# miaoyin390/DNN-Compression-Tensor-ADMM

Measured on AMD Instinct MI355X. Metric: ADMM projection iters/sec (all layers) + per-layer SVD GFLOP/s, ResNet-50 TT ranks, higher is better.
Workload: dtype f32 (Gram, eigen-solve and its filter products accumulate in f64); 1 GPU; resnet50_tt: 34 layers, 20099072 weights, hp table tt_resnet50_hp.HyperParamsDictGeneralRatio3x; tables=1, parallelism=layer-shard x1 (latency-model partition, one scalar all-reduce per step)

## Files before the change

### dnn-compression-tensor-admm_amd/csrc/filter.hip

```cpp
#include "common.h"

namespace tadmm {

typedef double double2v_t __attribute__((ext_vector_type(2)));
constexpr int kMomParts = 64;

__device__ __forceinline__ double hash_unit(uint32_t a, uint32_t b) {
  uint64_t x = ((uint64_t)a << 32) ^ (uint64_t)b;
  x += 0x9E3779B97F4A7C15ull;
  x = (x ^ (x >> 30)) * 0xBF58476D1CE4E5B9ull;
  x = (x ^ (x >> 27)) * 0x94D049BB133111EBull;
  x ^= x >> 31;
  return (double)(int64_t)(x >> 11) * (1.0 / 4503599627370496.0) - 1.0;
}

__global__ __launch_bounds__(256) void filt_init_kernel(const FiltProb* __restrict__ probs,
                                                        const BlockRef* __restrict__ map, int test_zero_col) {
  const BlockRef br = map[blockIdx.x];
  const FiltProb p = probs[br.prob];
  if (br.local == 0 && threadIdx.x == 0) {
    FiltState* st = p.st;
    st->base = 0; st->res = 1; st->nsteps = 0; st->active = 1; st->alive = 1; st->bad = 0; st->stage = 0;
    st->products = 2;
    st->products_fast = 0; st->precise_stages = 0; st->logamp_precise = 0.0;
// ... 4 lines not shown
  const int64_t total = (int64_t)p.rp * p.ldy;
  const int64_t i0 = ((int64_t)br.local * 256 + threadIdx.x) * 4;
  double* Y = p.ring[0];
#pragma unroll
  for (int u = 0; u < 4; ++u) {
    const int64_t i = i0 + u;
    if (i < total) {
      const int col = (int)(i % p.ldy);
      Y[i] = (col < p.N && col != test_zero_col) ? hash_unit((uint32_t)br.prob * 2654435761u + 17u, (uint32_t)i) : 0.0;
    }
  }
}

__device__ __forceinline__ double acosh_pos(double x) { return log(x + sqrt(fmax(x * x - 1.0, 0.0))); }

__global__ __launch_bounds__(256) void filt_plan_kernel(const FiltProb* __restrict__ probs, FiltParams prm,
                                                        int last_stage, int stage_fast, int* __restrict__ verdict) {
  __shared__ double rho[256], sorted[256];
  const FiltProb p = probs[blockIdx.x];
  FiltState* st = p.st;
  const int tid = threadIdx.x;
  if (st->bad || !st->active) {
    __syncthreads();
    if (tid == 0) {
      st->nsteps = 0; st->res = st->base; st->active = 0;
      if (st->bad) { st->alive = 0; *p.skip_slot = 1; }
      verdict[1 + blockIdx.x] = 0;
    }
    return;
  }
  const int rp = p.rp;
  for (int j = tid; j < rp; j += 256) {
    double v = 0.0;
    for (int t = 0; t < p.rq_tiles; ++t) v += p.rqpart[(int64_t)t * rp + j];
    rho[j] = v;
  }
  __syncthreads();
  for (int j = tid; j < rp; j += 256) {
    const double v = rho[j];
    int rank = 0;
    for (int i = 0; i < rp; ++i) {
      const double w = rho[i];
      rank += (w > v) || (w == v && i < j);
    }
    sorted[rank] = v;
  }
  __syncthreads();
  if (tid == 0) {
    const double l1 = sorted[0], lr = sorted[p.r - 1], b = sorted[rp - 1];
    bool ok = isfinite(l1) && isfinite(b) && b > 0.0 && lr > b * (1.0 + 1e-9) && l1 >= lr;
    int m = 0;
    bool more = false;
    if (ok) {
      const double e = 0.5 * b, c = 0.5 * b;
      const double xr = (lr - c) / e, x1 = (l1 - c) / e;
      const double ar = acosh_pos(xr), a1 = acosh_pos(x1);
      double need = prm.log_target - st->logamp;
      if (st->products_fast > 0 || (stage_fast & 1)) need = fmax(need, prm.log_precise - st->logamp_precise);
      if (need > 0.0) {
        const double ln2 = 0.6931471805599453;
        const double cmax = st->stage == 0 ? fmin(prm.cond_max, prm.cond_first) : prm.cond_max;
        int mc = (int)floor(log(2.0 * cmax) / a1);
        mc = max(1, mc);
        int mn = (int)ceil((need + ln2) / ar);
        mn = max(1, mn);
        m = min(prm.max_degree, min(mc, mn));
        st->logamp += m * ar - ln2;
        st->coef1[0] = 1.0 / e; st->coef1[1] = -c / e;
        st->coefk[0] = 2.0 / e; st->coefk[1] = -2.0 * c / e; st->coefk[2] = -1.0;
        if (!(stage_fast & 1)) { st->precise_stages += 1; st->logamp_precise += m * ar - ln2; }
        double after = prm.log_target - st->logamp;
        if (st->products_fast > 0 || (stage_fast & 1)) after = fmax(after, prm.log_precise - st->logamp_precise);
        more = after > 0.0;
      }
      st->b = b; st->lr = lr; st->l1 = l1;
    } else {
      st->bad = 1; st->alive = 0; *p.skip_slot = 1;
    }
    st->nsteps = m;
    st->products += (m > 0) ? m : 1;
    if (stage_fast & 1) st->products_fast += (m > 0) ? m : 1;
    if ((stage_fast & 2) && st->stage == 0) st->products_fast += 1;
    int res = st->base + m;
    res -= (res >= 3) ? 3 : 0; res -= (res >= 3) ? 3 : 0; res -= (res >= 3) ? 3 : 0;
    st->res = res % 3;
    st->active = (m > 0 && more && !last_stage) ? 1 : 0;
    st->stage += 1;
    verdict[1 + blockIdx.x] = (m > 0 ? 1 : 0) | (st->active ? 2 : 0);
  }
}

__global__ void filt_flags_kernel(const FiltProb* __restrict__ probs, int nprob) {
  const int q = blockIdx.x * blockDim.x + threadIdx.x;
  if (q >= nprob) return;
  const FiltProb p = probs[q];
  if (p.st->bad) { p.st->alive = 0; *p.skip_slot = 1; }
}

__global__ __launch_bounds__(256) void filt_theta_kernel(const FiltProb* __restrict__ probs) {
  const FiltProb p = probs[blockIdx.x];
  if (p.st->bad) return;
  for (int c = threadIdx.x; c < p.r32; c += 256) {
    const double s = c < p.r ? p.sigma[c] : 0.0;
    p.theta[c] = s * s;
  }
}

__global__ __launch_bounds__(256) void filt_verdict_kernel(const FiltProb* __restrict__ probs, FiltParams prm,
                                                           int* __restrict__ verdict) {
  __shared__ double part[256];
  const FiltProb p = probs[blockIdx.x];
  FiltState* st = p.st;
  const int tid = threadIdx.x;
  if (st->bad) {
    if (tid == 0) { verdict[1 + blockIdx.x] = 0; *p.fb_skip = 0; }
    return;
  }
  const double th_next = p.lam[p.order[p.r]];
  double acc = 0.0;
  for (int c = tid; c < p.r; c += 256) {
    double rn = 0.0;
    for (int t = 0; t < p.v_tiles; ++t) rn += p.vpart[(int64_t)t * p.r32 + c];
    const double gap = p.theta[c] - th_next;
    acc += (gap > 0.0) ? rn / (gap * gap) : INFINITY;
  }
  part[tid] = acc;
  __syncthreads();
  for (int o = 128; o > 0; o >>= 1) {
    if (tid < o) part[tid] += part[tid + o];
    __syncthreads();
  }
  if (tid == 0) {
    const double crit = sqrt(part[0]);
    st->crit = crit;
    const double th_r = p.theta[p.r - 1];
    bool guard_ok = !(st->guard > th_r * (1.0 + 1e-9)) && st->guard == st->guard;
    if (st->mom_on) {
      double m[5] = {0.0, 0.0, 0.0, 0.0, 0.0};
      for (int w = 0; w < kMomParts; ++w)
        for (int q = 0; q < 5; ++q) m[q] += st->mom[w * 5 + q];
      const double trd = m[1] - m[4], d2 = m[0] - 2.0 * m[2] + m[3];
      const double bound = trd > 0.0 ? d2 / trd : 0.0;
      if (bound > th_r * (1.0 + 1e-6) || bound != bound) guard_ok = false;
      st->guard = fmax(st->guard, bound);
    }
    const bool ok = crit <= prm.sin_tol && guard_ok;
    if (!ok) { st->bad = 1; st->alive = 0; }
    *p.fb_skip = ok ? 1 : 0;
    verdict[1 + blockIdx.x] = ok ? 1 : 0;
  }
}

__global__ __launch_bounds__(256) void filt_moments_kernel(const FiltProb* __restrict__ probs) {
  __shared__ double red[5][4];
  const FiltProb p = probs[blockIdx.x];
  FiltState* st = p.st;
  if (st->bad) return;
  const int part = blockIdx.y, tid = threadIdx.x, lane = tid & 63, wave = tid >> 6;
  int tb = st->base + 1;
  tb -= tb >= 3 ? 3 : 0;
  auto sumsq = [&](const double* __restrict__ a, int64_t total) {
    const int64_t per = ((total / kMomParts + 511) / 512) * 512;
    const int64_t lo = (int64_t)part * per, hi = lo + per < total ? lo + per : total;
    double s0 = 0.0, s1 = 0.0, s2 = 0.0, s3 = 0.0;
    for (int64_t i = lo + 2 * tid; i < hi; i += 2048) {
      double2v_t v0 = {0, 0}, v1 = {0, 0}, v2 = {0, 0}, v3 = {0, 0};
      v0 = *reinterpret_cast<const double2v_t*>(a + i);
      if (i + 512 < hi) v1 = *reinterpret_cast<const double2v_t*>(a + i + 512);
      if (i + 1024 < hi) v2 = *reinterpret_cast<const double2v_t*>(a + i + 1024);
      if (i + 1536 < hi) v3 = *reinterpret_cast<const double2v_t*>(a + i + 1536);
      s0 += v0.x * v0.x + v0.y * v0.y; s1 += v1.x * v1.x + v1.y * v1.y;
      s2 += v2.x * v2.x + v2.y * v2.y; s3 += v3.x * v3.x + v3.y * v3.y;
    }
    return (s0 + s1) + (s2 + s3);
  };
  const double g2 = sumsq(p.G, (int64_t)p.Npad * p.ldg);
  const double t2 = sumsq(p.ring[tb], (int64_t)p.rp * p.ldy);
  const double h2 = sumsq(p.H, (int64_t)p.rp * p.ldh);
  double tg = 0.0, th = 0.0;
  if (part == 0) {
    for (int i = tid; i < p.N; i += 256) tg += p.G[(int64_t)i * p.ldg + i];
    for (int j = tid; j < p.rp; j += 256) th += p.H[(int64_t)j * p.ldh + j];
  }
  double v[5] = {g2, tg, t2, h2, th};
#pragma unroll
  for (int q = 0; q < 5; ++q) {
#pragma unroll
    for (int o = 32; o > 0; o >>= 1) v[q] += __shfl_xor(v[q], o, 64);
    if (lane == 0) red[q][wave] = v[q];
  }
  __syncthreads();
  if (tid < 5) st->mom[part * 5 + tid] = (red[tid][0] + red[tid][1]) + (red[tid][2] + red[tid][3]);
  if (part == 0 && tid == 0) st->mom_on = 1;
}

__global__ __launch_bounds__(1024) void filt_guard_kernel(const FiltProb* __restrict__ probs, int nsteps) {
  extern __shared__ __attribute__((aligned(16))) double gsm[];
  __shared__ double red[16];
  const FiltProb p = probs[blockIdx.x];
  FiltState* st = p.st;
  if (st->bad) return;
  const int N = p.N, Npad = p.Npad, rp = p.rp, ldy = p.ldy, ldg = p.ldg;
  const double* __restrict__ Q = p.ring[st->base];
  const double* __restrict__ G = p.G;
  double* z = gsm;
  double* w = z + Npad;
  double* c = w + Npad;
  double* pacc = c + rp;
  const int tid = threadIdx.x, lane = tid & 63, wave = tid >> 6;
  auto wave_sum = [&](double v) {
#pragma unroll
    for (int o = 32; o > 0; o >>= 1) v += __shfl_xor(v, o, 64);
    return v;
  };
  auto block_sum = [&](double v) {
    v = wave_sum(v);
    __syncthreads();
    if (lane == 0) red[wave] = v;
// ... 81 lines not shown
    project(w);
    double a = 0.0, b = 0.0;
    for (int i = tid; i < N; i += 1024) { a += z[i] * w[i]; b += w[i] * w[i]; }
    rho = fmax(rho, block_sum(a));
    const double n2 = block_sum(b);
    if (!(n2 > 0.0)) break;
    const double inv = 1.0 / sqrt(n2);
    for (int i = tid; i < N; i += 1024) z[i] = w[i] * inv;
    __syncthreads();
  }
  if (tid == 0) st->guard = rho;
}

__global__ __launch_bounds__(256) void filt_emit_kernel(const FiltProb* __restrict__ probs,
                                                        const BlockRef* __restrict__ map) {
  const BlockRef br = map[blockIdx.x];
  const FiltProb p = probs[br.prob];
  if (p.st->bad) return;
  const int lane = threadIdx.x & 63, wave = threadIdx.x >> 6;
  const int c = br.local * 4 + wave;
  if (c >= p.r) return;
  const double* row = p.UT + (int64_t)c * p.ldy;
  const int N = p.N;
  double best = -1.0; int besti = 0;
  double nrm = 0.0;
  for (int i = lane; i < N; i += 64) {
    const double v = row[i], a = fabs(v);
    nrm += v * v;
    if (a > best) { best = a; besti = i; }
  }
#pragma unroll
  for (int o = 32; o > 0; o >>= 1) {
    const double ob = __shfl_down(best, o, 64);
    const int oi = __shfl_down(besti, o, 64);
    nrm += __shfl_xor(nrm, o, 64);
    if (ob > best || (ob == best && oi < besti)) { best = ob; besti = oi; }
  }
  besti = __shfl(besti, 0, 64);
  const double sgn = (row[besti] < 0.0) ? -1.0 : 1.0;
  const double inv = nrm > 0.0 ? sgn / sqrt(nrm) : 0.0;
  const double sig = p.sigma[c];
  const double isig = sig > 0.0 ? 1.0 / sig : 0.0;
  const int R = p.ldo ? p.ldo : p.r;
  for (int i = lane; i < N; i += 64) {
    const double v = row[i] * inv;
    if (p.mode == 0) {
      p.out_a[(int64_t)i * R + c] = (float)v;
    } else if (p.mode == 1) {
      p.out_a[(int64_t)i * R + c] = (float)(v * isig);
      p.out_b[(int64_t)c * N + i] = (float)(v * sig);
    } else if (p.mode == 3) {
      p.out_a[(int64_t)i * R + c] = (float)(v * isig);
    }
  }
}

void launch_filt_init(const FiltProb* probs_dev, const BlockRef* map_dev, int nblocks, int nprob, hipStream_t s) {
  if (nblocks <= 0) return;
  int zero_col = -1;
  if (const char* e = getenv("TADMM_FILTER_TEST_ZERO_COL")) zero_col = atoi(e);
  hipLaunchKernelGGL(filt_init_kernel, dim3(nblocks), dim3(256), 0, s, probs_dev, map_dev, zero_col);
}
void launch_filt_moments(const FiltProb* probs_dev, int nprob, hipStream_t s) {
  if (nprob <= 0) return;
  hipLaunchKernelGGL(filt_moments_kernel, dim3(nprob, kMomParts), dim3(256), 0, s, probs_dev);
}
void launch_filt_guard(const FiltProb* probs_dev, int nprob, int npad_max, int rp_max, int steps, hipStream_t s) {
// ... 28 lines not shown
```

### dnn-compression-tensor-admm_amd/csrc/filter_host.h

```cpp
#pragma once
#include <memory>
#include "host.h"

namespace tadmm {

static inline int filter_block_size(int N, int r) {
  const char* e = getenv("TADMM_FILTER");
  if (e && !atoi(e)) return 0;
  int min_n = 192;
  if (const char* m = getenv("TADMM_FILTER_MINN")) min_n = atoi(m);
  if (N < min_n || r < 16) return 0;
  double over = 1.45;
  if (const char* o = getenv("TADMM_FILTER_OVERSAMPLE")) over = atof(o);
  int rp = (int)align_up((size_t)(over * r + 0.999), 32);
  double min_over = 1.15;
  if (const char* o = getenv("TADMM_FILTER_MIN_OVERSAMPLE")) min_over = atof(o);
  if (rp > 256) {
    rp = 256;
    if ((double)rp < min_over * r) return 0;
  }
  if (rp * 100 > 56 * N || rp <= r) return 0;
  return rp;
}

// ... 495 lines not shown
    if (fg.side->ok && hipEventRecord(fg.side->fork, s) == hipSuccess &&
        hipStreamWaitEvent(fg.side->st, fg.side->fork, 0) == hipSuccess) {
      launch_filt_guard(probs, fg.nf, fg.npad_max, fg.rp_max, filter_guard_steps(), fg.side->st);
      fg.guard_forked = hipEventRecord(fg.side->join, fg.side->st) == hipSuccess;
    }
  }
  gemm(fg.tfinal);
  gemm(fg.hform);
  if (filter_moments_on()) launch_filt_moments(probs, fg.nf, s);
  if (debug) fprintf(stderr, "[tadmm] filter: %d problems, %d stages of <= %d steps, product tiles %d x %d (%d blocks a launch)\n", fg.nf, stages,
                     fg.max_degree, fg.tile_m, filter_tile_n(), fg.p1.nblocks);
  return TADMM_OK;
}

static inline int filter_run_post(tadmm_handle h, FilterGroup& fg, char* ws, PollCtx& poll, hipStream_t s, bool debug,
                                  int* nbad, FilterTiming* tm = nullptr) {
  *nbad = 0;
  if (fg.nf == 0) return TADMM_OK;
  auto D = [&](size_t off) { return ws + off; };
  const FiltProb* probs = (const FiltProb*)D(fg.prob_off);
  const FiltParams prm = filter_params(fg);
  launch_filt_theta(probs, fg.nf, s);
  if (fg.guard_forked) HIP_OK(h, hipStreamWaitEvent(s, fg.side->join, 0));
  else launch_filt_guard(probs, fg.nf, fg.npad_max, fg.rp_max, filter_guard_steps(), s);
  launch_dgemm((const DgemmDesc*)D(fg.uform.desc_off), (const BlockRef*)D(fg.uform.map_off), fg.uform.nblocks, false, s);
  {
    const bool t = tm && tm->on;
    if (t) (void)hipEventRecord(tm->a, s);
    launch_dgemm_nt64((const DgemmDesc*)D(fg.verify.desc_off), (const BlockRef*)D(fg.verify.map_off), fg.verify.nblocks, s, filter_tile_n(), fg.tile_m);
    if (t) {
      float ms = 0.f;
// ... 4 lines not shown
    }
  }
  if (fg.ncomp > 0) {
    const CompDesc* cd = (const CompDesc*)D(fg.comp_off);
    launch_comp_form(cd, (const BlockRef*)D(fg.cform.map_off), fg.cform.nblocks, s);
    for (int pass = 0; pass < 2; ++pass) {
      launch_dgemm_nt64((const DgemmDesc*)D(fg.cgram.desc_off), (const BlockRef*)D(fg.cgram.map_off), fg.cgram.nblocks, s, filter_tile_n(), fg.tile_m);
      launch_chol_factor((const CholDesc*)D(fg.cchol_off), fg.ncomp, s);
      launch_chol_solve((const CholDesc*)D(fg.cchol_off), (const BlockRef*)D(fg.csolve_map_off), fg.csolve_blocks, s);
    }
  }
  launch_filt_verdict(probs, fg.nf, prm, poll.host, s);
  launch_filt_emit(probs, (const BlockRef*)D(fg.emit.map_off), fg.emit.nblocks, s);
  if (fg.ncomp > 0) launch_comp_emit((const CompDesc*)D(fg.comp_off), (const BlockRef*)D(fg.cemit.map_off), fg.cemit.nblocks, s);
  HIP_OK(h, hipEventRecord(poll.ev[0], s));
  HIP_OK(h, hipEventSynchronize(poll.ev[0]));
  int bad = 0;
  for (int q = 0; q < fg.nf; ++q) bad += poll.host[1 + q] ? 0 : 1;
  *nbad = bad;
  fg.last_bad = bad;
  if (tm && tm->on) {
    std::vector<FiltProb> hp(fg.nf);
    if (hipMemcpy(hp.data(), probs, hp.size() * sizeof(FiltProb), hipMemcpyDeviceToHost) == hipSuccess) {
      for (int q = 0; q < fg.nf; ++q) {
        FiltState st;
        if (hipMemcpy(&st, hp[q].st, sizeof st, hipMemcpyDeviceToHost) != hipSuccess) break;
        const double rp = hp[q].rp, np = hp[q].Npad, r32 = hp[q].r32;
        const double stages = st.stage;
        tm->fast_flops += 2.0 * rp * np * np * st.products_fast;
        tm->gemm_flops += 2.0 * rp * np * np * (st.products - st.products_fast)
// ... 22 lines not shown
```

### dnn-compression-tensor-admm_amd/csrc/gram.hip

```cpp
#include "common.h"
#include <type_traits>

namespace tadmm {

typedef double double4_t __attribute__((ext_vector_type(4)));

__device__ __forceinline__ double4_t mfma_f64(double a, double b, double4_t c) {
  return __builtin_amdgcn_mfma_f64_16x16x4f64(a, b, c, 0, 0, 0);
}

__device__ __forceinline__ void tile_pair(int tp, int nt, int& ti, int& tj) {
  int a = 0, rowlen = nt;
  while (tp >= rowlen) { tp -= rowlen; ++a; --rowlen; }
  ti = a; tj = a + tp;
}

__global__ __launch_bounds__(256) void gram_partial_kernel(const GramDesc* __restrict__ descs,
                                                           const BlockRef* __restrict__ map,
                                                           const int32_t* __restrict__ skip) {
  __shared__ double red[4][4][64 * 4];
  __shared__ double tile[32][33];
  const BlockRef br = map[blockIdx.x];
  if (skip && skip[br.prob]) return;
  const GramDesc d = descs[br.prob];
// ... 148 lines not shown
    G[(int64_t)(ti * 32 + rr) * gld + tj * 32 + cc] = tile[rr][cc];
    if (!diag) G[(int64_t)(tj * 32 + rr) * gld + ti * 32 + cc] = tile[cc][rr];
  }
  if (tj == d.nt - 1) {
    const int padw = d.ld - d.Npad;
    for (int e = threadIdx.x; e < 32 * padw; e += 256) {
      const int rr = e / padw, cc = e - rr * padw;
      G[(int64_t)(ti * 32 + rr) * gld + d.Npad + cc] = 0.0;
    }
  }
}

__global__ __launch_bounds__(256) void gram_reduce_kernel(const GramDesc* __restrict__ descs,
                                                          const BlockRef* __restrict__ map,
                                                          const int32_t* __restrict__ skip) {
  const BlockRef br = map[blockIdx.x];
  if (skip && skip[br.prob]) return;
  const GramDesc d = descs[br.prob];
  const int ntp = d.nt * (d.nt + 1) / 2;
  const int64_t total = (int64_t)d.Npad * d.ld;
  const int64_t base = (int64_t)br.local * 1024;
  for (int t = threadIdx.x; t < 1024; t += 256) {
    const int64_t idx = base + t;
    if (idx >= total) break;
    const int j = (int)(idx / d.ld), i = (int)(idx - (int64_t)j * d.ld);
    double v = 0.0;
    if (j < d.N && i < d.N) {
      int a = j >> 5, b = i >> 5, jr = j & 31, ir = i & 31;
      if (a > b) { int s = a; a = b; b = s; s = jr; jr = ir; ir = s; }
      if (a == b && jr > ir) { const int s = jr; jr = ir; ir = s; }
      const int tp = a * d.nt - (a * (a - 1)) / 2 + (b - a);
      const double* p = d.partial + (int64_t)tp * 1024 + jr * 32 + ir;
      const int64_t stride = (int64_t)ntp * 1024;
      int ks = 0;
      for (; ks + 8 <= d.ksplit; ks += 8) {
        double t[8];
#pragma unroll
        for (int u = 0; u < 8; ++u) t[u] = p[(ks + u) * stride];
        v += ((t[0] + t[1]) + (t[2] + t[3])) + ((t[4] + t[5]) + (t[6] + t[7]));
      }
      for (; ks < d.ksplit; ++ks) v += p[ks * stride];
    }
    d.G[idx] = v;
  }
}

void launch_gram_partial(const GramDesc* descs_dev, const BlockRef* map_dev, int nblocks, hipStream_t s,
                         const int32_t* skip) {
  if (nblocks <= 0) return;
  hipLaunchKernelGGL(gram_partial_kernel, dim3(nblocks), dim3(256), 0, s, descs_dev, map_dev, skip);
}

void launch_gram_reduce(const GramDesc* descs_dev, const BlockRef* map_dev, int nblocks, hipStream_t s,
                        const int32_t* skip) {
  if (nblocks <= 0) return;
  hipLaunchKernelGGL(gram_reduce_kernel, dim3(nblocks), dim3(256), 0, s, descs_dev, map_dev, skip);
}

// ... 2 lines not shown
```

### dnn-compression-tensor-admm_amd/csrc/host.h

```cpp
#pragma once
#include "common.h"

#include <algorithm>
#include <atomic>
#include <cstdio>
#include <cstdlib>
#include <cstring>
#include <functional>
#include <string>
#include <vector>

struct tadmm_ctx_s {
  int device = 0;
  std::string err;
};

#define CTX_FAIL(h, code, ...)                                   \
  do {                                                           \
    char _b[512];                                                \
    snprintf(_b, sizeof _b, __VA_ARGS__);                        \
    if (h) (h)->err = _b;                                        \
    return (code);                                               \
  } while (0)

// ... 242 lines not shown
  int gsteps = 0;
  EigTick kernel = EigTick::Pairs;
  int ld_max = 0;
  size_t tick_lds = 0;
  const BlockRef* tick_map = nullptr; int tick_blocks = 0;
  const BlockRef* self_map = nullptr; int self_blocks = 0;
  double* prev_dev = nullptr;
  const int32_t* skip = nullptr;
  int npad_max = 0;
  int expected = 0;
  bool aligned = false;
  bool warm = false;
  const int* row_len = nullptr;
  const int* mid_sizes = nullptr;
  std::function<void(hipStream_t)> after_init;
  const double* off_dev = nullptr; const int* done_dev = nullptr;
};

struct EigLayout {
  Phase tick, self, norm, ext;
  std::vector<int> players;
  std::vector<int> row_len;
  std::vector<int> mid;
  int neig = 0;
  int gsteps = 0;
  EigTick kernel = EigTick::Pairs;
  int ld_max = 0, npad_max = 0;
  size_t tick_lds = 0;
  bool aligned = false;
  size_t prev_off = 0;
// ... 58 lines not shown
}

static inline int build_eig_layout(tadmm_handle h, EigLayout& l, std::vector<EigDesc>& descs, bool align, Arena& da,
                                   HostImage* img) {
  EigMaps m;
  const int rc = eig_maps(h, l, descs, align, m);
  if (rc != TADMM_OK) return rc;
  place_phase(l.tick, da, img, descs.data(), descs.size() * sizeof(EigDesc), l.neig, m.tick);
  place_map_like(l.self, l.tick, da, img, m.self);
  place_map_like(l.norm, l.tick, da, img, m.norm);
  place_map_like(l.ext, l.tick, da, img, m.ext);
  return TADMM_OK;
}

static inline int run_eig_group(tadmm_handle h, const EigGroup& g, PollCtx& poll, double tol, int max_sweeps, bool debug,
                                hipStream_t s, int* sweeps_out, bool* small_pending, JacobiTiming* jt = nullptr) {
  const bool super = g.kernel == EigTick::SuperPairs;
  *sweeps_out = 0;
  *small_pending = false;
  if (g.neig == 0) return TADMM_OK;
  {
    const char* e = getenv("TADMM_JACOBI_SMALL");
    if (g.npad_max > 0 && jacobi_small_fits(g.npad_max) && !(e && !atoi(e))) {
      const bool timed = jt && jt->on;
      if (timed) (void)hipEventRecord(jt->a, s);
      int32_t* fast = (g.prev_dev && eig_small_direct_on()) ? reinterpret_cast<int32_t*>(g.prev_dev) : nullptr;
      if (fast) HIP_OK(h, launch_eig_small_direct(g.ed, g.neig, g.skip, fast, poll.host, s));
      HIP_OK(h, launch_jacobi_small(g.ed, g.neig, g.npad_max, tol, std::max(max_sweeps, 60), g.skip, poll.host, s, g.warm, fast));
      if (timed) {
        float ms = 0.f;
        (void)hipEventRecord(jt->b, s);
        (void)hipEventSynchronize(jt->b);
        (void)hipEventElapsedTime(&ms, jt->a, jt->b);
        jt->small_ms += ms; jt->small_launches += 1;
// ... 86 lines not shown
      for (int q = 0; q < g.neig; ++q) {
        const int steps = g.players[q] - 1;
        if (h_done[q]) ++nd;
        if (steps > 0 && tick % steps == 0) mxo = std::max(mxo, h_off[3 * q + ((tick / steps - 1) & 1)]);
      }
      fprintf(stderr, "[tadmm]   sweep %d: max observed off %.3e, done %d/%d\n", gs, mxo, nd, g.neig);
    }
    int rc = consume();
    if (rc != TADMM_OK) CTX_FAIL(h, rc, "poll event failed");
    if (all_done) break;
    static const bool lazy_poll = !(getenv("TADMM_POLL_EVERY_SWEEP") && atoi(getenv("TADMM_POLL_EVERY_SWEEP")));
    if (lazy_poll && !(jt && jt->on) && g.expected > 0 && gs + 3 < g.expected) continue;
    HIP_OK(h, hipEventRecord(poll.ev[gs & 1], s));
    pending = gs;
    if (g.expected > 0 && gs + 1 >= g.expected) {
      rc = consume();
      if (rc != TADMM_OK) CTX_FAIL(h, rc, "poll event failed");
    }
  }
  if (!all_done) {
    const int rc = consume();
    if (rc != TADMM_OK) CTX_FAIL(h, rc, "poll event failed");
  }
  if (debug) {
    int pmax = 0;
    for (int q = 0; q < g.neig; ++q) pmax = std::max(pmax, g.players[q]);
    fprintf(stderr, "[tadmm] eig group: neig=%d players_max=%d ticks/sweep=%d wgs/tick=%d sweeps=%d ticks=%d kernel=%s\n",
            g.neig, pmax, g.gsteps, g.tick_blocks, all_done ? needed : gs, tick, super ? "super-pairs" : "pairs");
  }
  if (!all_done) CTX_FAIL(h, TADMM_ERR_NOCONVERGE, "Jacobi did not converge in %d sweeps", max_sweeps);
  *sweeps_out = needed;
  return TADMM_OK;
}

static inline int check_small_group(tadmm_handle h, const EigGroup& g, PollCtx& poll) {
  if (hipEventSynchronize(poll.ev[0]) != hipSuccess) CTX_FAIL(h, TADMM_ERR_HIP, "poll event failed");
  for (int q = 0; q < g.neig; ++q)
    if (!poll.host[1 + q]) CTX_FAIL(h, TADMM_ERR_NOCONVERGE, "Jacobi (small problems) did not converge, problem %d", q);
  return TADMM_OK;
}

}
```

### dnn-compression-tensor-admm_amd/csrc/plan.hip

```cpp
#include "host.h"
#include "filter_host.h"

#include <cmath>
#include <condition_variable>
#include <mutex>
#include <thread>

using namespace tadmm;

struct StepGeom : EigGeom {
  StepGeom() = default;
  explicit StepGeom(const EigGeom& g) : EigGeom(g) {}
  int r = 0;
  bool skip = false;
};

struct LayerGeom {
  tadmm_layer_desc desc;
  int64_t numel = 0;
  int O = 0, I = 0, K2 = 1;
  int d = 0;
  std::vector<StepGeom> steps;
};

// ... 57 lines not shown
      CTX_FAIL(h, TADMM_ERR_UNSUPPORTED, "TT step %d: eigen-problem of size %d exceeds the Jacobi kernels (max %d)", s,
               st.N, kJacobiMaxN);
  }
  return TADMM_OK;
}

struct StepPlan {
  Phase gram_p, gram_r, proj;
  EigLayout main, fb;
  size_t off_off = 0, done_off = 0;
  std::vector<int> layer_of;
  FilterGroup fg;
  std::vector<int> filt_of;
  size_t skip_off = 0;
  size_t fb_skip_off = 0;
};

struct tadmm_plan_s {
  tadmm_handle h = nullptr;
  int n = 0;
  std::vector<LayerGeom> layers;
  char* ws = nullptr;
  size_t ws_bytes = 0;
  Phase unfold, fold;
  size_t sweep_desc_off = 0;
  size_t resid_partial_off = 0;
  int total_sweep_blocks = 0;
  std::vector<StepPlan> steps;
  std::vector<Phase> recon;
  std::vector<std::vector<size_t>> sigma_off;
  bool timing = false;
// ... 273 lines not shown
      filter_layout(sp.fg, fspecs, da, ar, dev, img, rr);
      for (int i = 0; i < nf; ++i) {
        const int p = sp.filt_of[i];
        ed_fb.push_back(ed[p]);
        ed_fb.back().off = (double*)dev(ar.take(3 * 8));
        ed_fb.back().done = (int32_t*)dev(ar.take(4));
        EigDesc e = rr[i].desc;
        e.off = ed[p].off; e.done = ed[p].done;
        ed[p] = e;
      }
    }
    if (const int rc = build_eig_layout(h, sp.main, ed, true, da, img)) return rc;
    sp.fb.prev_off = ar.take((size_t)std::max<size_t>(1, ed_fb.size()) * 8);
    if (const int rc = build_eig_layout(h, sp.fb, ed_fb, true, da, img)) return rc;
    place_phase(sp.proj, da, img, pd.data(), pd.size() * sizeof(GemmDesc), neig, m_proj);
  }

  for (int l = 0; l < n; ++l) lastT[l] = cur[l];
  size_t maxchain = 0;
  for (int l = 0; l < n; ++l) maxchain = std::max(maxchain, recops[l].size());
  P->recon.assign(maxchain, Phase());
  std::vector<const float*> rcur(n);
  std::vector<float*> rfree(n);
  for (int l = 0; l < n; ++l) {
    rcur[l] = lastT[l];
    float* b0 = (float*)dev(tb0[l]);
    float* b1 = (float*)dev(tb1[l]);
    rfree[l] = (rcur[l] == b0) ? b1 : b0;
  }
  for (size_t lev = 0; lev < maxchain; ++lev) {
// ... 412 lines not shown
  auto tic = [&](int i) { if (p->timing) (void)hipEventRecord(p->ev[i], s); };
  auto toc = [&](int i, int slot) {
    if (!p->timing) return;
    (void)hipEventRecord(p->ev[i + 1], s);
    (void)hipEventSynchronize(p->ev[i + 1]);
    float ms = 0.f;
    (void)hipEventElapsedTime(&ms, p->ev[i], p->ev[i + 1]);
    acc_ms[slot] += ms;
  };

  tic(0);
  launch_unfold((const SweepDesc*)D(p->sweep_desc_off), (const BlockRef*)D(p->unfold.map_off), p->unfold.nblocks,
                use_u, s);
  toc(0, 0);

  auto solve_group = [&](EigLayout& L, const EigGroup& eg, bool* small_pending) -> int {
    int gs = 0;
    const int rc = run_eig_group(h, eg, p->poll, p->tol, p->max_global_sweeps, p->debug, s, &gs,
                                 small_pending, &p->jtm);
    if (rc != TADMM_OK) return rc;
    L.last_sweeps = gs;
    total_sweeps += gs;
    L.finalize(ws, s, eg.skip);
    return TADMM_OK;
  };

  for (StepPlan& sp : p->steps) {
    if (sp.main.neig == 0) continue;
    tic(0);
    launch_gram_partial((const GramDesc*)D(sp.gram_p.desc_off), (const BlockRef*)D(sp.gram_p.map_off),
                        sp.gram_p.nblocks, s);
    launch_gram_reduce((const GramDesc*)D(sp.gram_r.desc_off), (const BlockRef*)D(sp.gram_r.map_off),
                       sp.gram_r.nblocks, s);
    toc(0, 1);
    tic(0);
    const bool filtered = sp.fg.nf > 0;
    if (filtered) {
      const int rc = filter_run_pre(h, sp.fg, ws, p->poll, s, p->debug, &p->ftm);
      if (rc != TADMM_OK) return rc;
    }
    EigGroup eg = sp.main.group(ws, filtered ? (const int32_t*)D(sp.skip_off) : nullptr);
    eg.off_dev = (const double*)D(sp.off_off); eg.done_dev = (const int*)D(sp.done_off);
    eg.expected = sp.main.last_sweeps;
    bool small_pending = false;
    {
      const int rc = solve_group(sp.main, eg, &small_pending);
      if (rc != TADMM_OK) return rc;
    }
    if (filtered) {
      if (small_pending) {
        const int rc = check_small_group(h, eg, p->poll);
        if (rc != TADMM_OK) return rc;
        small_pending = false;
      }
      int nbad = 0;
      int rc = filter_run_post(h, sp.fg, ws, p->poll, s, p->debug, &nbad, &p->ftm);
      if (rc != TADMM_OK) return rc;
      p->filt_problems += sp.fg.nf;
      p->filt_fallbacks += nbad;
      p->filt_stages = std::max(p->filt_stages, sp.fg.last_stages);
      if (nbad > 0) {
        const EigGroup fgp = sp.fb.group(ws, (const int32_t*)D(sp.fb_skip_off));
        bool fsmall = false;
        rc = solve_group(sp.fb, fgp, &fsmall);
        if (rc != TADMM_OK) return rc;
        if (fsmall) {
          rc = check_small_group(h, fgp, p->poll);
          if (rc != TADMM_OK) return rc;
        }
      }
    }
    toc(0, 2);
    tic(0);
    launch_gemm((const GemmDesc*)D(sp.proj.desc_off), (const BlockRef*)D(sp.proj.map_off), sp.proj.nblocks, s);
    toc(0, 3);
    if (small_pending) {
      const int rc = check_small_group(h, eg, p->poll);
      if (rc != TADMM_OK) return rc;
    }
  }
  tic(0);
  for (Phase& ph : p->recon)
    launch_gemm((const GemmDesc*)D(ph.desc_off), (const BlockRef*)D(ph.map_off), ph.nblocks, s);
  toc(0, 4);
  tic(0);
  double* partial = (double*)D(p->resid_partial_off);
  launch_fold_update((const SweepDesc*)D(p->sweep_desc_off), (const BlockRef*)D(p->fold.map_off), p->fold.nblocks,
                     update_u, partial, s);
  if (resid_sq_dev)
// ... 82 lines not shown
```

Baseline: 170.9 iters/s.

## Prefetch filter state, vectorize reductions, and speculatively enqueue projection and finalize

```diff
diff --git a/dnn-compression-tensor-admm_amd/csrc/filter.hip b/dnn-compression-tensor-admm_amd/csrc/filter.hip
--- a/dnn-compression-tensor-admm_amd/csrc/filter.hip
+++ b/dnn-compression-tensor-admm_amd/csrc/filter.hip
@@ -42,40 +42,67 @@
 
 __device__ __forceinline__ double acosh_pos(double x) { return log(x + sqrt(fmax(x * x - 1.0, 0.0))); }
 
+typedef const G<const FiltProb>* FiltProbPtr;
+
+__device__ __forceinline__ double* filt_ring(FiltProbPtr pp, int i) {
+  double* r0 = pp->ring[0]; double* r1 = pp->ring[1]; double* r2 = pp->ring[2];
+  return i == 0 ? +r0 : (i == 1 ? +r1 : +r2);
+}
+
+__device__ __forceinline__ double sum16_in_order(double v, const G<const double>* col, int64_t ld, int n) {
+  double x[16];
+#pragma unroll
+  for (int u = 0; u < 16; ++u) x[u] = col[(int64_t)min(u, n - 1) * ld];
+#pragma unroll
+  for (int u = 0; u < 16; ++u) v = u < n ? v + x[u] : v;
+  return v;
+}
+
 __global__ __launch_bounds__(256) void filt_plan_kernel(const FiltProb* __restrict__ probs, FiltParams prm,
                                                         int last_stage, int stage_fast, int* __restrict__ verdict) {
-  __shared__ double rho[256], sorted[256];
-  const FiltProb p = probs[blockIdx.x];
-  FiltState* st = p.st;
+  __shared__ __attribute__((aligned(16))) double rho[256];
+  __shared__ double sorted[256];
+  FiltProbPtr pp = gp(probs + blockIdx.x);
+  G<FiltState>* st = gp(pp->st);
+  const G<const double>* rq = gp(pp->rqpart);
+  G<int32_t>* skip_slot = gp(pp->skip_slot);
+  G<int32_t>* vd = gp(verdict) + 1 + blockIdx.x;
+  const int rp = pp->rp, r = pp->r, rq_tiles = pp->rq_tiles;
   const int tid = threadIdx.x;
-  if (st->bad || !st->active) {
+  const int s_bad = st->bad, s_active = st->active, s_base = st->base, s_stage = st->stage;
+  const int s_products = st->products, s_products_fast = st->products_fast, s_precise_stages = st->precise_stages;
+  const double s_logamp = st->logamp, s_logamp_precise = st->logamp_precise;
+  double v0 = 0.0;
+  if (rq_tiles > 0) v0 = sum16_in_order(v0, rq + min(tid, rp - 1), rp, min(rq_tiles, 16));
+  if (s_bad || !s_active) {
     __syncthreads();
     if (tid == 0) {
-      st->nsteps = 0; st->res = st->base; st->active = 0;
-      if (st->bad) { st->alive = 0; *p.skip_slot = 1; }
-      verdict[1 + blockIdx.x] = 0;
+      st->nsteps = 0; st->res = s_base; st->active = 0;
+      if (s_bad) { st->alive = 0; *skip_slot = 1; }
+      *vd = 0;
     }
     return;
   }
-  const int rp = p.rp;
   for (int j = tid; j < rp; j += 256) {
-    double v = 0.0;
-    for (int t = 0; t < p.rq_tiles; ++t) v += p.rqpart[(int64_t)t * rp + j];
+    double v = j == tid ? v0 : 0.0;
+    for (int t = j == tid ? 16 : 0; t < rq_tiles; t += 16)
+      v = sum16_in_order(v, rq + (int64_t)t * rp + j, rp, min(rq_tiles - t, 16));
     rho[j] = v;
   }
   __syncthreads();
   for (int j = tid; j < rp; j += 256) {
     const double v = rho[j];
     int rank = 0;
-    for (int i = 0; i < rp; ++i) {
-      const double w = rho[i];
-      rank += (w > v) || (w == v && i < j);
+    for (int i = 0; i < rp; i += 2) {
+      const double2v_t w = *reinterpret_cast<const double2v_t*>(&rho[i]);
+      rank += (w.x > v) || (w.x == v && i < j);
+      rank += (w.y > v) || (w.y == v && i + 1 < j);
     }
     sorted[rank] = v;
   }
   __syncthreads();
   if (tid == 0) {
-    const double l1 = sorted[0], lr = sorted[p.r - 1], b = sorted[rp - 1];
+    const double l1 = sorted[0], lr = sorted[r - 1], b = sorted[rp - 1];
     bool ok = isfinite(l1) && isfinite(b) && b > 0.0 && lr > b * (1.0 + 1e-9) && l1 >= lr;
     int m = 0;
     bool more = false;
@@ -83,38 +110,46 @@
       const double e = 0.5 * b, c = 0.5 * b;
       const double xr = (lr - c) / e, x1 = (l1 - c) / e;
       const double ar = acosh_pos(xr), a1 = acosh_pos(x1);
-      double need = prm.log_target - st->logamp;
-      if (st->products_fast > 0 || (stage_fast & 1)) need = fmax(need, prm.log_precise - st->logamp_precise);
+      double need = prm.log_target - s_logamp;
+      if (s_products_fast > 0 || (stage_fast & 1)) need = fmax(need, prm.log_precise - s_logamp_precise);
       if (need > 0.0) {
         const double ln2 = 0.6931471805599453;
-        const double cmax = st->stage == 0 ? fmin(prm.cond_max, prm.cond_first) : prm.cond_max;
+        const double cmax = s_stage == 0 ? fmin(prm.cond_max, prm.cond_first) : prm.cond_max;
         int mc = (int)floor(log(2.0 * cmax) / a1);
         mc = max(1, mc);
         int mn = (int)ceil((need + ln2) / ar);
         mn = max(1, mn);
         m = min(prm.max_degree, min(mc, mn));
-        st->logamp += m * ar - ln2;
+        double logamp = s_logamp, logamp_precise = s_logamp_precise;
+        logamp += m * ar - ln2;
+        st->logamp = logamp;
         st->coef1[0] = 1.0 / e; st->coef1[1] = -c / e;
         st->coefk[0] = 2.0 / e; st->coefk[1] = -2.0 * c / e; st->coefk[2] = -1.0;
-        if (!(stage_fast & 1)) { st->precise_stages += 1; st->logamp_precise += m * ar - ln2; }
-        double after = prm.log_target - st->logamp;
-        if (st->products_fast > 0 || (stage_fast & 1)) after = fmax(after, prm.log_precise - st->logamp_precise);
+        if (!(stage_fast & 1)) {
+          logamp_precise += m * ar - ln2;
+          st->precise_stages = s_precise_stages + 1; st->logamp_precise = logamp_precise;
+        }
+        double after = prm.log_target - logamp;
+        if (s_products_fast > 0 || (stage_fast & 1)) after = fmax(after, prm.log_precise - logamp_precise);
         more = after > 0.0;
       }
       st->b = b; st->lr = lr; st->l1 = l1;
     } else {
-      st->bad = 1; st->alive = 0; *p.skip_slot = 1;
+      st->bad = 1; st->alive = 0; *skip_slot = 1;
     }
     st->nsteps = m;
-    st->products += (m > 0) ? m : 1;
-    if (stage_fast & 1) st->products_fast += (m > 0) ? m : 1;
-    if ((stage_fast & 2) && st->stage == 0) st->products_fast += 1;
-    int res = st->base + m;
+    st->products = s_products + ((m > 0) ? m : 1);
+    int products_fast = s_products_fast;
+    if (stage_fast & 1) products_fast += (m > 0) ? m : 1;
+    if ((stage_fast & 2) && s_stage == 0) products_fast += 1;
+    if ((stage_fast & 1) || ((stage_fast & 2) && s_stage == 0)) st->products_fast = products_fast;
+    int res = s_base + m;
     res -= (res >= 3) ? 3 : 0; res -= (res >= 3) ? 3 : 0; res -= (res >= 3) ? 3 : 0;
     st->res = res % 3;
-    st->active = (m > 0 && more && !last_stage) ? 1 : 0;
-    st->stage += 1;
-    verdict[1 + blockIdx.x] = (m > 0 ? 1 : 0) | (st->active ? 2 : 0);
+    const int active = (m > 0 && more && !last_stage) ? 1 : 0;
+    st->active = active;
+    st->stage = s_stage + 1;
+    *vd = (m > 0 ? 1 : 0) | (active ? 2 : 0);
   }
 }
 
@@ -136,20 +171,37 @@
 
 __global__ __launch_bounds__(256) void filt_verdict_kernel(const FiltProb* __restrict__ probs, FiltParams prm,
                                                            int* __restrict__ verdict) {
-  __shared__ double part[256];
-  const FiltProb p = probs[blockIdx.x];
-  FiltState* st = p.st;
+  __shared__ double part[256], mom[kMomParts * 5];
+  FiltProbPtr pp = gp(probs + blockIdx.x);
+  G<FiltState>* st = gp(pp->st);
+  G<int32_t>* fb_skip = gp(pp->fb_skip);
+  G<int32_t>* vd = gp(verdict) + 1 + blockIdx.x;
+  const G<const double>* theta = gp((const double*)pp->theta);
+  const G<const double>* vpart = gp(pp->vpart);
+  const int r = pp->r, r32 = pp->r32, v_tiles = pp->v_tiles;
   const int tid = threadIdx.x;
-  if (st->bad) {
-    if (tid == 0) { verdict[1 + blockIdx.x] = 0; *p.fb_skip = 0; }
+  const int s_bad = st->bad, s_mom_on = st->mom_on;
+  const double s_guard = st->guard;
+  const int inext = gp(pp->order)[r];
+  const double th_r = theta[r - 1];
+  const int c0 = min(tid, r - 1);
+  const double th_c0 = theta[c0];
+  double rn0 = 0.0;
+  if (v_tiles > 0) rn0 = sum16_in_order(rn0, vpart + c0, r32, min(v_tiles, 16));
+  const double mom_a = st->mom[tid], mom_b = st->mom[256 + (tid & 63)];
+  if (s_bad) {
+    if (tid == 0) { *vd = 0; *fb_skip = 0; }
     return;
   }
-  const double th_next = p.lam[p.order[p.r]];
+  const double th_next = gp(pp->lam)[inext];
+  mom[tid] = mom_a;
+  if (tid < kMomParts * 5 - 256) mom[256 + tid] = mom_b;
   double acc = 0.0;
-  for (int c = tid; c < p.r; c += 256) {
-    double rn = 0.0;
-    for (int t = 0; t < p.v_tiles; ++t) rn += p.vpart[(int64_t)t * p.r32 + c];
-    const double gap = p.theta[c] - th_next;
+  for (int c = tid; c < r; c += 256) {
+    double rn = c == tid ? rn0 : 0.0;
+    for (int t = c == tid ? 16 : 0; t < v_tiles; t += 16)
+      rn = sum16_in_order(rn, vpart + (int64_t)t * r32 + c, r32, min(v_tiles - t, 16));
+    const double gap = (c == tid ? th_c0 : theta[c]) - th_next;
     acc += (gap > 0.0) ? rn / (gap * gap) : INFINITY;
   }
   part[tid] = acc;
@@ -161,54 +213,95 @@
   if (tid == 0) {
     const double crit = sqrt(part[0]);
     st->crit = crit;
-    const double th_r = p.theta[p.r - 1];
-    bool guard_ok = !(st->guard > th_r * (1.0 + 1e-9)) && st->guard == st->guard;
-    if (st->mom_on) {
+    bool guard_ok = !(s_guard > th_r * (1.0 + 1e-9)) && s_guard == s_guard;
+    if (s_mom_on) {
       double m[5] = {0.0, 0.0, 0.0, 0.0, 0.0};
       for (int w = 0; w < kMomParts; ++w)
-        for (int q = 0; q < 5; ++q) m[q] += st->mom[w * 5 + q];
+        for (int q = 0; q < 5; ++q) m[q] += mom[w * 5 + q];
       const double trd = m[1] - m[4], d2 = m[0] - 2.0 * m[2] + m[3];
       const double bound = trd > 0.0 ? d2 / trd : 0.0;
       if (bound > th_r * (1.0 + 1e-6) || bound != bound) guard_ok = false;
-      st->guard = fmax(st->guard, bound);
+      st->guard = fmax(s_guard, bound);
     }
     const bool ok = crit <= prm.sin_tol && guard_ok;
     if (!ok) { st->bad = 1; st->alive = 0; }
-    *p.fb_skip = ok ? 1 : 0;
-    verdict[1 + blockIdx.x] = ok ? 1 : 0;
+    *fb_skip = ok ? 1 : 0;
+    *vd = ok ? 1 : 0;
   }
 }
 
 __global__ __launch_bounds__(256) void filt_moments_kernel(const FiltProb* __restrict__ probs) {
   __shared__ double red[5][4];
-  const FiltProb p = probs[blockIdx.x];
-  FiltState* st = p.st;
-  if (st->bad) return;
+  FiltProbPtr pp = gp(probs + blockIdx.x);
+  G<FiltState>* st = gp(pp->st);
+  const int s_bad = st->bad, s_base = st->base;
+  const int N = pp->N, Npad = pp->Npad, rp = pp->rp, ldy = pp->ldy, ldg = pp->ldg, ldh = pp->ldh;
+  const G<const double>* Gm = gp(pp->G);
+  const G<const double>* Hm = gp(pp->H);
+  if (s_bad) return;
   const int part = blockIdx.y, tid = threadIdx.x, lane = tid & 63, wave = tid >> 6;
-  int tb = st->base + 1;
+  int tb = s_base + 1;
   tb -= tb >= 3 ? 3 : 0;
-  auto sumsq = [&](const double* __restrict__ a, int64_t total) {
+  const G<const double>* Tm = gp((const double*)filt_ring(pp, tb));
+  struct Slice { const G<const double>* a; int64_t i, hi; double2v_t v[4]; };
+  auto slice_load = [](Slice& s) {
+#pragma unroll
+    for (int k = 0; k < 4; ++k) {
+      const int64_t e = s.i + 512 * k;
+      s.v[k] = *reinterpret_cast<const G<const double2v_t>*>(s.a + (e < s.hi ? e : 0));
+    }
+  };
+  auto slice_open = [&](const G<const double>* a, int64_t total) {
     const int64_t per = ((total / kMomParts + 511) / 512) * 512;
-    const int64_t lo = (int64_t)part * per, hi = lo + per < total ? lo + per : total;
+    const int64_t lo = (int64_t)part * per;
+    Slice s;
+    s.a = a; s.i = lo + 2 * tid; s.hi = lo + per < total ? lo + per : total;
+    slice_load(s);
+    return s;
+  };
+  auto slice_sum = [&](Slice& s) {
     double s0 = 0.0, s1 = 0.0, s2 = 0.0, s3 = 0.0;
-    for (int64_t i = lo + 2 * tid; i < hi; i += 2048) {
-      double2v_t v0 = {0, 0}, v1 = {0, 0}, v2 = {0, 0}, v3 = {0, 0};
-      v0 = *reinterpret_cast<const double2v_t*>(a + i);
-      if (i + 512 < hi) v1 = *reinterpret_cast<const double2v_t*>(a + i + 512);
-      if (i + 1024 < hi) v2 = *reinterpret_cast<const double2v_t*>(a + i + 1024);
-      if (i + 1536 < hi) v3 = *reinterpret_cast<const double2v_t*>(a + i + 1536);
+    for (;;) {
+      const double2v_t zero = {0, 0};
+      const double2v_t v0 = s.i < s.hi ? s.v[0] : zero, v1 = s.i + 512 < s.hi ? s.v[1] : zero;
+      const double2v_t v2 = s.i + 1024 < s.hi ? s.v[2] : zero, v3 = s.i + 1536 < s.hi ? s.v[3] : zero;
       s0 += v0.x * v0.x + v0.y * v0.y; s1 += v1.x * v1.x + v1.y * v1.y;
       s2 += v2.x * v2.x + v2.y * v2.y; s3 += v3.x * v3.x + v3.y * v3.y;
+      s.i += 2048;
+      if (!(s.i < s.hi)) break;
+      slice_load(s);
     }
     return (s0 + s1) + (s2 + s3);
   };
-  const double g2 = sumsq(p.G, (int64_t)p.Npad * p.ldg);
-  const double t2 = sumsq(p.ring[tb], (int64_t)p.rp * p.ldy);
-  const double h2 = sumsq(p.H, (int64_t)p.rp * p.ldh);
+  Slice sg = slice_open(Gm, (int64_t)Npad * ldg);
+  Slice st2 = slice_open(Tm, (int64_t)rp * ldy);
+  Slice sh = slice_open(Hm, (int64_t)rp * ldh);
+  auto diag_load = [&](const G<const double>* a, int ld, int n, int i0, double (&d)[4]) {
+#pragma unroll
+    for (int k = 0; k < 4; ++k) {
+      const int i = i0 + 256 * k;
+      d[k] = a[i < n ? (int64_t)i * ld + i : 0];
+    }
+  };
+  auto diag_add = [&](double t, int n, int i0, const double (&d)[4]) {
+#pragma unroll
+    for (int k = 0; k < 4; ++k) t = i0 + 256 * k < n ? t + d[k] : t;
+    return t;
+  };
+  double dg[4] = {0.0, 0.0, 0.0, 0.0}, dh[4] = {0.0, 0.0, 0.0, 0.0};
+  if (part == 0) {
+    diag_load(Gm, ldg, N, tid, dg);
+    diag_load(Hm, ldh, rp, tid, dh);
+  }
+  const double g2 = slice_sum(sg);
+  const double t2 = slice_sum(st2);
+  const double h2 = slice_sum(sh);
   double tg = 0.0, th = 0.0;
   if (part == 0) {
-    for (int i = tid; i < p.N; i += 256) tg += p.G[(int64_t)i * p.ldg + i];
-    for (int j = tid; j < p.rp; j += 256) th += p.H[(int64_t)j * p.ldh + j];
+    tg = diag_add(tg, N, tid, dg);
+    for (int i0 = tid + 1024; i0 < N; i0 += 1024) { diag_load(Gm, ldg, N, i0, dg); tg = diag_add(tg, N, i0, dg); }
+    th = diag_add(th, rp, tid, dh);
+    for (int j0 = tid + 1024; j0 < rp; j0 += 1024) { diag_load(Hm, ldh, rp, j0, dh); th = diag_add(th, rp, j0, dh); }
   }
   double v[5] = {g2, tg, t2, h2, th};
 #pragma unroll
@@ -229,7 +322,9 @@
   FiltState* st = p.st;
   if (st->bad) return;
   const int N = p.N, Npad = p.Npad, rp = p.rp, ldy = p.ldy, ldg = p.ldg;
-  const double* __restrict__ Q = p.ring[st->base];
+  const int qb = st->base;
+  const double* q0 = +p.ring[0]; const double* q1 = +p.ring[1]; const double* q2 = +p.ring[2];
+  const double* __restrict__ Q = qb == 0 ? +q0 : (qb == 1 ? +q1 : +q2);
   const double* __restrict__ G = p.G;
   double* z = gsm;
   double* w = z + Npad;
@@ -341,43 +436,66 @@
 
 __global__ __launch_bounds__(256) void filt_emit_kernel(const FiltProb* __restrict__ probs,
                                                         const BlockRef* __restrict__ map) {
-  const BlockRef br = map[blockIdx.x];
-  const FiltProb p = probs[br.prob];
-  if (p.st->bad) return;
-  const int lane = threadIdx.x & 63, wave = threadIdx.x >> 6;
-  const int c = br.local * 4 + wave;
-  if (c >= p.r) return;
-  const double* row = p.UT + (int64_t)c * p.ldy;
-  const int N = p.N;
-  double best = -1.0; int besti = 0;
+  const G<const BlockRef>* br = gp(map + blockIdx.x);
+  const int prob = br->prob, local = br->local;
+  FiltProbPtr pp = gp(probs + prob);
+  const int s_bad = gp(pp->st)->bad;
+  const int N = pp->N, r = pp->r, ldy = pp->ldy, ldo = pp->ldo, mode = pp->mode;
+  G<float>* out_a = gp(pp->out_a);
+  G<float>* out_b = gp(pp->out_b);
+  const int lane = threadIdx.x & 63, wave = __builtin_amdgcn_readfirstlane(threadIdx.x >> 6);
+  const int c = local * 4 + wave;
+  if (c >= r) return;
+  const G<const double>* row = gp(pp->UT) + (int64_t)c * ldy;
+  const double sig = gp((const double*)pp->sigma)[c];
+  double x[8];
+  auto row_load = [&](int i0) {
+#pragma unroll
+    for (int k = 0; k < 8; ++k) x[k] = row[min(i0 + 64 * k, N - 1)];
+  };
+  row_load(lane);
+  if (s_bad) return;
+  double best = -1.0, bestv = 0.0; int besti = 0;
   double nrm = 0.0;
-  for (int i = lane; i < N; i += 64) {
-    const double v = row[i], a = fabs(v);
-    nrm += v * v;
-    if (a > best) { best = a; besti = i; }
+  for (int i0 = lane; i0 < N; i0 += 512) {
+    if (i0 != lane) row_load(i0);
+#pragma unroll
+    for (int k = 0; k < 8; ++k) {
+      const int i = i0 + 64 * k;
+      if (i < N) {
+        const double v = x[k], a = fabs(v);
+        nrm += v * v;
+        if (a > best) { best = a; besti = i; bestv = v; }
+      }
+    }
   }
 #pragma unroll
   for (int o = 32; o > 0; o >>= 1) {
-    const double ob = __shfl_down(best, o, 64);
+    const double ob = __shfl_down(best, o, 64), ov = __shfl_down(bestv, o, 64);
     const int oi = __shfl_down(besti, o, 64);
     nrm += __shfl_xor(nrm, o, 64);
-    if (ob > best || (ob == best && oi < besti)) { best = ob; besti = oi; }
-  }
-  besti = __shfl(besti, 0, 64);
-  const double sgn = (row[besti] < 0.0) ? -1.0 : 1.0;
+    if (ob > best || (ob == best && oi < besti)) { best = ob; besti = oi; bestv = ov; }
+  }
+  bestv = __shfl(bestv, 0, 64);
+  const double sgn = (bestv < 0.0) ? -1.0 : 1.0;
   const double inv = nrm > 0.0 ? sgn / sqrt(nrm) : 0.0;
-  const double sig = p.sigma[c];
   const double isig = sig > 0.0 ? 1.0 / sig : 0.0;
-  const int R = p.ldo ? p.ldo : p.r;
-  for (int i = lane; i < N; i += 64) {
-    const double v = row[i] * inv;
-    if (p.mode == 0) {
-      p.out_a[(int64_t)i * R + c] = (float)v;
-    } else if (p.mode == 1) {
-      p.out_a[(int64_t)i * R + c] = (float)(v * isig);
-      p.out_b[(int64_t)c * N + i] = (float)(v * sig);
-    } else if (p.mode == 3) {
-      p.out_a[(int64_t)i * R + c] = (float)(v * isig);
+  const int R = ldo ? ldo : r;
+  for (int i0 = lane; i0 < N; i0 += 512) {
+    if (N > 512) row_load(i0);
+#pragma unroll
+    for (int k = 0; k < 8; ++k) {
+      const int i = i0 + 64 * k;
+      if (i >= N) continue;
+      const double v = x[k] * inv;
+      if (mode == 0) {
+        out_a[(int64_t)i * R + c] = (float)v;
+      } else if (mode == 1) {
+        out_a[(int64_t)i * R + c] = (float)(v * isig);
+        out_b[(int64_t)c * N + i] = (float)(v * sig);
+      } else if (mode == 3) {
+        out_a[(int64_t)i * R + c] = (float)(v * isig);
+      }
     }
   }
 }
diff --git a/dnn-compression-tensor-admm_amd/csrc/filter_host.h b/dnn-compression-tensor-admm_amd/csrc/filter_host.h
--- a/dnn-compression-tensor-admm_amd/csrc/filter_host.h
+++ b/dnn-compression-tensor-admm_amd/csrc/filter_host.h
@@ -533,7 +533,8 @@
 }
 
 static inline int filter_run_post(tadmm_handle h, FilterGroup& fg, char* ws, PollCtx& poll, hipStream_t s, bool debug,
-                                  int* nbad, FilterTiming* tm = nullptr) {
+                                  int* nbad, FilterTiming* tm = nullptr,
+                                  const std::function<void()>& behind_verdict = nullptr) {
   *nbad = 0;
   if (fg.nf == 0) return TADMM_OK;
   auto D = [&](size_t off) { return ws + off; };
@@ -568,6 +569,7 @@
   launch_filt_emit(probs, (const BlockRef*)D(fg.emit.map_off), fg.emit.nblocks, s);
   if (fg.ncomp > 0) launch_comp_emit((const CompDesc*)D(fg.comp_off), (const BlockRef*)D(fg.cemit.map_off), fg.cemit.nblocks, s);
   HIP_OK(h, hipEventRecord(poll.ev[0], s));
+  if (behind_verdict) behind_verdict();
   HIP_OK(h, hipEventSynchronize(poll.ev[0]));
   int bad = 0;
   for (int q = 0; q < fg.nf; ++q) bad += poll.host[1 + q] ? 0 : 1;
diff --git a/dnn-compression-tensor-admm_amd/csrc/gram.hip b/dnn-compression-tensor-admm_amd/csrc/gram.hip
--- a/dnn-compression-tensor-admm_amd/csrc/gram.hip
+++ b/dnn-compression-tensor-admm_amd/csrc/gram.hip
@@ -186,34 +186,60 @@
 __global__ __launch_bounds__(256) void gram_reduce_kernel(const GramDesc* __restrict__ descs,
                                                           const BlockRef* __restrict__ map,
                                                           const int32_t* __restrict__ skip) {
-  const BlockRef br = map[blockIdx.x];
-  if (skip && skip[br.prob]) return;
-  const GramDesc d = descs[br.prob];
-  const int ntp = d.nt * (d.nt + 1) / 2;
-  const int64_t total = (int64_t)d.Npad * d.ld;
-  const int64_t base = (int64_t)br.local * 1024;
-  for (int t = threadIdx.x; t < 1024; t += 256) {
-    const int64_t idx = base + t;
-    if (idx >= total) break;
-    const int j = (int)(idx / d.ld), i = (int)(idx - (int64_t)j * d.ld);
-    double v = 0.0;
-    if (j < d.N && i < d.N) {
-      int a = j >> 5, b = i >> 5, jr = j & 31, ir = i & 31;
-      if (a > b) { int s = a; a = b; b = s; s = jr; jr = ir; ir = s; }
-      if (a == b && jr > ir) { const int s = jr; jr = ir; ir = s; }
-      const int tp = a * d.nt - (a * (a - 1)) / 2 + (b - a);
-      const double* p = d.partial + (int64_t)tp * 1024 + jr * 32 + ir;
-      const int64_t stride = (int64_t)ntp * 1024;
-      int ks = 0;
-      for (; ks + 8 <= d.ksplit; ks += 8) {
-        double t[8];
-#pragma unroll
-        for (int u = 0; u < 8; ++u) t[u] = p[(ks + u) * stride];
-        v += ((t[0] + t[1]) + (t[2] + t[3])) + ((t[4] + t[5]) + (t[6] + t[7]));
-      }
-      for (; ks < d.ksplit; ++ks) v += p[ks * stride];
-    }
-    d.G[idx] = v;
+  const G<const BlockRef>* brp = gp(map + blockIdx.x);
+  const int prob = brp->prob, local = brp->local;
+  const G<const GramDesc>* d = gp(descs + prob);
+  const int nt = d->nt, N = d->N, Npad = d->Npad, ld = d->ld, ksplit = d->ksplit;
+  const G<const double>* partial = gp((const double*)d->partial);
+  G<double>* Gout = gp(d->G);
+  if (skip && gp(skip)[prob]) return;
+  const int ntp = nt * (nt + 1) / 2;
+  const int64_t total = (int64_t)Npad * ld;
+  const int64_t base = (int64_t)local * 1024;
+  const int64_t stride = (int64_t)ntp * 1024;
+  const bool small = total <= 0x7fffffff;
+  const G<const double>* p[4];
+  bool live[4];
+  double v[4] = {0.0, 0.0, 0.0, 0.0};
+#pragma unroll
+  for (int o = 0; o < 4; ++o) {
+    const int64_t idx = base + threadIdx.x + 256 * o;
+    const int j = small ? (int)((uint32_t)idx / (uint32_t)ld) : (int)(idx / ld);
+    const int i = (int)(idx - (int64_t)j * ld);
+    live[o] = idx < total && j < N && i < N;
+    int a = j >> 5, b = i >> 5, jr = j & 31, ir = i & 31;
+    if (a > b) { int s = a; a = b; b = s; s = jr; jr = ir; ir = s; }
+    if (a == b && jr > ir) { const int s = jr; jr = ir; ir = s; }
+    const int tp = a * nt - (a * (a - 1)) / 2 + (b - a);
+    p[o] = live[o] ? partial + (int64_t)tp * 1024 + jr * 32 + ir : partial;
+  }
+  int ks = 0;
+  for (; ks + 8 <= ksplit; ks += 8) {
+    double t[4][8];
+#pragma unroll
+    for (int o = 0; o < 4; ++o)
+#pragma unroll
+      for (int u = 0; u < 8; ++u) t[o][u] = p[o][(ks + u) * stride];
+#pragma unroll
+    for (int o = 0; o < 4; ++o)
+      v[o] += ((t[o][0] + t[o][1]) + (t[o][2] + t[o][3])) + ((t[o][4] + t[o][5]) + (t[o][6] + t[o][7]));
+  }
+  if (ks < ksplit) {
+    double t[4][7];
+    const int n = ksplit - ks;
+#pragma unroll
+    for (int o = 0; o < 4; ++o)
+#pragma unroll
+      for (int u = 0; u < 7; ++u) t[o][u] = p[o][(ks + min(u, n - 1)) * stride];
+#pragma unroll
+    for (int o = 0; o < 4; ++o)
+#pragma unroll
+      for (int u = 0; u < 7; ++u) v[o] = u < n ? v[o] + t[o][u] : v[o];
+  }
+#pragma unroll
+  for (int o = 0; o < 4; ++o) {
+    const int64_t idx = base + threadIdx.x + 256 * o;
+    if (idx < total) Gout[idx] = live[o] ? v[o] : 0.0;
   }
 }
 
diff --git a/dnn-compression-tensor-admm_amd/csrc/host.h b/dnn-compression-tensor-admm_amd/csrc/host.h
--- a/dnn-compression-tensor-admm_amd/csrc/host.h
+++ b/dnn-compression-tensor-admm_amd/csrc/host.h
@@ -280,6 +280,7 @@
   const int* row_len = nullptr;
   const int* mid_sizes = nullptr;
   std::function<void(hipStream_t)> after_init;
+  std::function<void(hipStream_t)> behind_last;
   const double* off_dev = nullptr; const int* done_dev = nullptr;
 };
 
@@ -368,10 +369,13 @@
 }
 
 static inline int run_eig_group(tadmm_handle h, const EigGroup& g, PollCtx& poll, double tol, int max_sweeps, bool debug,
-                                hipStream_t s, int* sweeps_out, bool* small_pending, JacobiTiming* jt = nullptr) {
+                                hipStream_t s, int* sweeps_out, bool* small_pending, JacobiTiming* jt = nullptr,
+                                bool* behind_last_stands = nullptr) {
   const bool super = g.kernel == EigTick::SuperPairs;
   *sweeps_out = 0;
   *small_pending = false;
+  if (behind_last_stands) *behind_last_stands = false;
+  bool stands = false;
   if (g.neig == 0) return TADMM_OK;
   {
     const char* e = getenv("TADMM_JACOBI_SMALL");
@@ -488,8 +492,10 @@
     HIP_OK(h, hipEventRecord(poll.ev[gs & 1], s));
     pending = gs;
     if (g.expected > 0 && gs + 1 >= g.expected) {
+      if (g.behind_last && behind_last_stands) { g.behind_last(s); stands = true; }
       rc = consume();
       if (rc != TADMM_OK) CTX_FAIL(h, rc, "poll event failed");
+      if (!all_done) stands = false;
     }
   }
   if (!all_done) {
@@ -504,6 +510,7 @@
   }
   if (!all_done) CTX_FAIL(h, TADMM_ERR_NOCONVERGE, "Jacobi did not converge in %d sweeps", max_sweeps);
   *sweeps_out = needed;
+  if (behind_last_stands) *behind_last_stands = stands;
   return TADMM_OK;
 }
 
diff --git a/dnn-compression-tensor-admm_amd/csrc/plan.hip b/dnn-compression-tensor-admm_amd/csrc/plan.hip
--- a/dnn-compression-tensor-admm_amd/csrc/plan.hip
+++ b/dnn-compression-tensor-admm_amd/csrc/plan.hip
@@ -95,7 +95,22 @@
   std::vector<int> filt_of;
   size_t skip_off = 0;
   size_t fb_skip_off = 0;
+  bool proj_repeatable = false;
 };
+
+static inline void gemm_span(const float* p, int64_t rows, int64_t cols, int64_t rs, int64_t cs, const float** lo, const float** hi) {
+  *lo = p;
+  *hi = p + (rows - 1) * rs + (cols - 1) * cs + 1;
+}
+static inline bool gemm_repeatable(const GemmDesc& g) {
+  if (g.beta != 0.f || g.M <= 0 || g.N <= 0 || g.K <= 0) return false;
+  if (g.a_rs < 0 || g.a_cs < 0 || g.b_rs < 0 || g.b_cs < 0 || g.c_rs < 0 || g.c_cs < 0) return false;
+  const float *c0, *c1, *a0, *a1, *b0, *b1;
+  gemm_span(g.C, g.M, g.N, g.c_rs, g.c_cs, &c0, &c1);
+  gemm_span(g.A, g.M, g.K, g.a_rs, g.a_cs, &a0, &a1);
+  gemm_span(g.B, g.K, g.N, g.b_rs, g.b_cs, &b0, &b1);
+  return (c1 <= a0 || a1 <= c0) && (c1 <= b0 || b1 <= c0);
+}
 
 struct tadmm_plan_s {
   tadmm_handle h = nullptr;
@@ -399,6 +414,8 @@
     sp.fb.prev_off = ar.take((size_t)std::max<size_t>(1, ed_fb.size()) * 8);
     if (const int rc = build_eig_layout(h, sp.fb, ed_fb, true, da, img)) return rc;
     place_phase(sp.proj, da, img, pd.data(), pd.size() * sizeof(GemmDesc), neig, m_proj);
+    sp.proj_repeatable = !pd.empty();
+    for (const GemmDesc& g : pd) sp.proj_repeatable = sp.proj_repeatable && gemm_repeatable(g);
   }
 
   for (int l = 0; l < n; ++l) lastT[l] = cur[l];
@@ -841,14 +858,16 @@
                 use_u, s);
   toc(0, 0);
 
-  auto solve_group = [&](EigLayout& L, const EigGroup& eg, bool* small_pending) -> int {
+  auto solve_group = [&](EigLayout& L, EigGroup eg, bool* small_pending) -> int {
     int gs = 0;
+    bool finalized = false;
+    eg.behind_last = [&](hipStream_t st) { L.finalize(ws, st, eg.skip); };
     const int rc = run_eig_group(h, eg, p->poll, p->tol, p->max_global_sweeps, p->debug, s, &gs,
-                                 small_pending, &p->jtm);
+                                 small_pending, &p->jtm, &finalized);
     if (rc != TADMM_OK) return rc;
     L.last_sweeps = gs;
     total_sweeps += gs;
-    L.finalize(ws, s, eg.skip);
+    if (!finalized) L.finalize(ws, s, eg.skip);
     return TADMM_OK;
   };
 
@@ -870,6 +889,10 @@
     eg.off_dev = (const double*)D(sp.off_off); eg.done_dev = (const int*)D(sp.done_off);
     eg.expected = sp.main.last_sweeps;
     bool small_pending = false;
+    bool proj_queued = false;
+    auto launch_proj = [&] {
+      launch_gemm((const GemmDesc*)D(sp.proj.desc_off), (const BlockRef*)D(sp.proj.map_off), sp.proj.nblocks, s);
+    };
     {
       const int rc = solve_group(sp.main, eg, &small_pending);
       if (rc != TADMM_OK) return rc;
@@ -881,8 +904,12 @@
         small_pending = false;
       }
       int nbad = 0;
-      int rc = filter_run_post(h, sp.fg, ws, p->poll, s, p->debug, &nbad, &p->ftm);
+      std::function<void()> early_proj;
+      if (sp.proj_repeatable && !p->timing)
+        early_proj = [&] { launch_proj(); proj_queued = true; };
+      int rc = filter_run_post(h, sp.fg, ws, p->poll, s, p->debug, &nbad, &p->ftm, early_proj);
       if (rc != TADMM_OK) return rc;
+      if (nbad > 0) proj_queued = false;
       p->filt_problems += sp.fg.nf;
       p->filt_fallbacks += nbad;
       p->filt_stages = std::max(p->filt_stages, sp.fg.last_stages);
@@ -899,7 +926,7 @@
     }
     toc(0, 2);
     tic(0);
-    launch_gemm((const GemmDesc*)D(sp.proj.desc_off), (const BlockRef*)D(sp.proj.map_off), sp.proj.nblocks, s);
+    if (!proj_queued) launch_proj();
     toc(0, 3);
     if (small_pending) {
       const int rc = check_small_group(h, eg, p->poll);
```

Result: faster. 174.1 iters/s (median of 6 runs) (+1.9%).
